# Arash-san/YinYang-Game-AlphaZero

Hardware: AMD Instinct MI355X
Metric: self-play positions/sec (+ MCTS node-expansions/sec) at 800 sims, 8x8 board (higher is better)
Workload: dtype f16x3; 1 GPU; 8x8 board, 800 sims/move, 4096 concurrent games per GPU, frozen random-init 128x10 net (seed 0), copied boards, reference_quirks=False, staggered start plies; tree_arithmetic=f32 PUCT + u64 bitboards, nn_dtype=f16x3, evaluation_reuse=False, parallelism=episode-sharded x1, lanes_per_gpu=2, hipgraph=True

## Files before the change

include/yy_engine.h:

```cpp
#ifndef YY_ENGINE_H
#define YY_ENGINE_H

#include <stdint.h>

#ifdef __cplusplus
extern "C" {
#endif

#define YY_OK 0
#define YY_E_INVALID (-1)
#define YY_E_UNSUPPORTED (-2)
#define YY_E_NOMEM (-3)
#define YY_E_HIP (-4)
#define YY_E_STATE (-5)
#define YY_E_ARENA (-6)

#define YY_FLAG_ROWCOL 1u
#define YY_FLAG_ALIASED 2u
#define YY_FLAG_REUSE_PASS_VALUE 4u

#define YY_FLAG_REUSE_TRANSPOSITIONS 8u
#define YY_FLAG_KEEP_EVALUATIONS 16u

typedef void *yy_stream_t;
// ... 59 lines not shown
int yy_mcts_root_counts(yy_mcts *ctx, int32_t *counts, float *child_w, float *child_p,
                        yy_stream_t stream);

int yy_mcts_root_policy(yy_mcts *ctx, int temperature_is_zero, double *pi, yy_stream_t stream);

int yy_mcts_root_stats(yy_mcts *ctx, int32_t *visits, double *value_sum, yy_stream_t stream);

int yy_mcts_get_boards(yy_mcts *ctx, int8_t *boards, yy_stream_t stream);

int yy_mcts_status(yy_mcts *ctx, int32_t *n_overflow, uint64_t *counters);
int yy_mcts_reset_counters(yy_mcts *ctx, yy_stream_t stream);
int yy_book_insert(const uint64_t *keys, int n, int R, int C, uint32_t *meta, uint64_t *table_keys, int64_t cap,
                   int32_t *slot_of, yy_stream_t stream);
int yy_mcts_set_book(yy_mcts *ctx, const uint32_t *meta, const uint64_t *keys, const float *value, const float *policy,
                     int64_t cap, int max_stones);
int yy_mcts_cache_clear(yy_mcts *ctx, yy_stream_t stream);

int yy_nn_bias_act_bf16(void *x, const float *bias, const void *residual, int64_t rows, int C,
                        int relu, yy_stream_t stream);

int yy_nn_tower_bf16(const float *planes, const void *weights, const float *bias, void *out, int G,
                     int R, int C, int channels, int n_layers, yy_stream_t stream);

int yy_nn_tower_heads_bf16(const float *planes, const void *weights, const float *bias,
                           void *out_heads, int G, int R, int C, int channels, int n_layers,
                           yy_stream_t stream);

int yy_nn_tower_f32(const float *planes, const void *weights, const float *bias, float *out, int G,
                    int R, int C, int channels, int n_layers, yy_stream_t stream);

int yy_nn_head_finish_bf16(const void *h, int G, int A, int H, const float *w2, const float *b2,
                           float *policy, float *value, yy_stream_t stream);

int yy_nn_tower_f16x3_regs(const float *planes, const void *weights, const void *head_w, const float *bias,
                           float *out, float *out_heads, const int32_t *rows, const int32_t *n_rows, int G,
                           int R, int C, int channels, int n_layers, int weight_exp, int head_exp,
                           int act_exp, yy_stream_t stream);

int yy_nn_tower_g(const float *planes, const void *weights, const void *head_w, const float *bias, const float *head_bias,
                  float *out, float *out_heads, const int32_t *rows, const int32_t *n_rows, int G, int R, int C,
                  int channels, int n_layers, int weight_exp, int head_exp, int act_exp, int nb, int boards, int gate_lo,
                  int gate_hi, int layout, yy_stream_t stream);
int yy_nn_tower_g_forms(int channels, int *nb_out);
int yy_nn_tower_g_relu_check(uint32_t start, uint32_t count, uint32_t *counts, yy_stream_t stream);

int yy_nn_fc_heads_f16x3(const float *feats, const void *wpk, const float *bias, const int32_t *jobs, int n_jobs,
                         float *logits, float *hidden, const int32_t *n_rows, int G, int K, int A, int H,
                         int weight_exp, int act_exp, yy_stream_t stream);

int yy_nn_head_finish_f32(const float *logits, const float *hidden, int G, int A, int H, const float *w2,
                          const float *b2, const int32_t *rows, const int32_t *n_rows, float *policy,
                          float *value, yy_stream_t stream);

int yy_compact_rows(const uint8_t *flags, int G, int32_t *rows, int32_t *n, yy_stream_t stream);

int yy_selfplay_root_noise(uint64_t seed, const int64_t *game_id, const int32_t *ply, const uint8_t *draw,
                           const uint8_t *mask, int G, int A, double alpha, double *noise, yy_stream_t stream);

int yy_selfplay_sample_actions(uint64_t seed, const int64_t *game_id, const int32_t *ply,
                               const uint8_t *searching, const double *pi, const uint8_t *mask, int G, int A,
                               int temperature_threshold, int32_t *action, yy_stream_t stream);

#ifdef __cplusplus
}
#endif
#endif
```

yinyang-game-alphazero_amd/_lib.py:

```python
import ctypes as C
import os
import subprocess

_HERE = os.path.dirname(os.path.abspath(__file__))
CSRC = os.path.join(_HERE, "csrc")
SO = os.path.join(CSRC, "libyy_hip.so")
HEADER = os.path.normpath(os.path.join(_HERE, "..", "include", "yy_engine.h"))

YY_OK = 0
YY_E_ARENA = -6
FLAG_ROWCOL = 1
FLAG_ALIASED = 2
FLAG_REUSE_PASS_VALUE = 4
FLAG_REUSE_TRANSPOSITIONS = 8
FLAG_KEEP_EVALUATIONS = 16

HIPCC_FLAGS = ["--offload-arch=gfx950", "-O3", "-std=c++17", "-fPIC", "-shared",
               "-ffp-contract=off", "-fno-fast-math", "-Wall", "-Wno-unused-function"]


class YYError(RuntimeError):
    def __init__(self, code, msg):
        super().__init__(f"libyy_hip: status {code}: {msg}")
        self.code = code
# ... 17 lines not shown
    if verbose:
        print(" ".join(cmd).replace(tmp, SO))
    try:
        subprocess.check_call(cmd)
        os.replace(tmp, SO)
    finally:
        if os.path.exists(tmp):
            os.remove(tmp)
    return SO


_LIB = None
_vp = C.c_void_p
_SIGS = {
    "yy_rules_valid_mask": [_vp, _vp, C.c_int, C.c_int, C.c_int, C.c_uint32, _vp, _vp],
    "yy_rules_step": [_vp, _vp, _vp, C.c_int, C.c_int, C.c_int, C.c_uint32, _vp, _vp],
    "yy_rules_game_ended": [_vp, _vp, C.c_int, C.c_int, C.c_int, C.c_uint32, _vp, _vp, _vp],
    "yy_encode_planes": [_vp, C.c_int, C.c_int, C.c_int, _vp, _vp],
    "yy_rules_mask_terminal_bb": [_vp, _vp, C.c_int, C.c_int, C.c_int, C.c_uint32, _vp, _vp, _vp, _vp],
    "yy_pack_boards": [_vp, C.c_int, C.c_int, C.c_int, _vp, _vp, _vp],
    "yy_unpack_boards": [_vp, _vp, C.c_int, C.c_int, C.c_int, _vp, _vp],
    "yy_mcts_create": [C.POINTER(MctsConfig), C.POINTER(_vp)],
    "yy_mcts_destroy": [_vp],
    "yy_mcts_memory_bytes": [_vp, C.POINTER(C.c_uint64)],
    "yy_mcts_set_num_sims": [_vp, C.c_int32],
    "yy_mcts_begin": [_vp, _vp, _vp, _vp, _vp, _vp],
    "yy_mcts_expand_root": [_vp, _vp, _vp, C.c_double, _vp],
    "yy_mcts_select": [_vp, _vp, _vp, _vp],
    "yy_mcts_expand_backup": [_vp, _vp, _vp, _vp],
    "yy_mcts_step": [_vp, _vp, _vp, _vp, _vp, _vp],
    "yy_mcts_root_counts": [_vp, _vp, _vp, _vp, _vp],
    "yy_mcts_root_policy": [_vp, C.c_int, _vp, _vp],
    "yy_mcts_root_stats": [_vp, _vp, _vp, _vp],
    "yy_mcts_get_boards": [_vp, _vp, _vp],
    "yy_mcts_status": [_vp, C.POINTER(C.c_int32), C.POINTER(C.c_uint64)],
    "yy_mcts_reset_counters": [_vp, _vp],
    "yy_mcts_cache_clear": [_vp, _vp],
    "yy_book_insert": [_vp, C.c_int, C.c_int, C.c_int, _vp, _vp, C.c_int64, _vp, _vp],
    "yy_mcts_set_book": [_vp, _vp, _vp, _vp, _vp, C.c_int64, C.c_int],
    "yy_nn_bias_act_bf16": [_vp, _vp, _vp, C.c_int64, C.c_int, C.c_int, _vp],
    "yy_nn_tower_bf16": [_vp, _vp, _vp, _vp, C.c_int, C.c_int, C.c_int, C.c_int, C.c_int, _vp],
    "yy_nn_tower_heads_bf16": [_vp, _vp, _vp, _vp, C.c_int, C.c_int, C.c_int, C.c_int, C.c_int, _vp],
    "yy_nn_head_finish_bf16": [_vp, C.c_int, C.c_int, C.c_int, _vp, _vp, _vp, _vp, _vp],
    "yy_nn_tower_f32": [_vp, _vp, _vp, _vp, C.c_int, C.c_int, C.c_int, C.c_int, C.c_int, _vp],
    "yy_nn_head_finish_f32": [_vp, _vp, C.c_int, C.c_int, C.c_int, _vp, _vp, _vp, _vp, _vp, _vp, _vp],
    "yy_compact_rows": [_vp, C.c_int, _vp, _vp, _vp],
    "yy_nn_tower_f16x3_regs": [_vp, _vp, _vp, _vp, _vp, _vp, _vp, _vp, C.c_int, C.c_int, C.c_int, C.c_int, C.c_int, C.c_int, C.c_int,
                               C.c_int, _vp],
    "yy_nn_tower_g_forms": [C.c_int, C.POINTER(C.c_int)],
    "yy_nn_tower_g_relu_check": [C.c_uint32, C.c_uint32, _vp, _vp],
    "yy_nn_tower_g": [_vp, _vp, _vp, _vp, _vp, _vp, _vp, _vp, _vp, C.c_int, C.c_int, C.c_int, C.c_int, C.c_int, C.c_int, C.c_int,
                      C.c_int, C.c_int, C.c_int, C.c_int, C.c_int, C.c_int, _vp],
    "yy_nn_fc_heads_f16x3": [_vp, _vp, _vp, _vp, C.c_int, _vp, _vp, _vp, C.c_int, C.c_int, C.c_int, C.c_int, C.c_int, C.c_int, _vp],
    "yy_selfplay_root_noise": [C.c_uint64, _vp, _vp, _vp, _vp, C.c_int, C.c_int, C.c_double, _vp, _vp],
    "yy_selfplay_sample_actions": [C.c_uint64, _vp, _vp, _vp, _vp, _vp, C.c_int, C.c_int, C.c_int, _vp, _vp],
    "yy_version": [],
}


def exported_symbols():
    return sorted(list(_SIGS) + ["yy_last_error"])


def lib():
    global _LIB
    if _LIB is None:
        if not os.path.exists(SO):
            raise YYError(-100, f"{SO} is missing: run __graft_entry__.build() (hipcc --offload-arch=gfx950); "
                                "there is no CPU fallback for the product path")
        L = C.CDLL(SO)
        for name, args in _SIGS.items():
            fn = getattr(L, name)
            fn.argtypes = args
            fn.restype = C.c_int
        L.yy_last_error.restype = C.c_char_p
        L.yy_last_error.argtypes = []
        _LIB = L
    return _LIB


def check(status):
    if status != YY_OK:
        raise YYError(status, lib().yy_last_error().decode())
    return status
```

yinyang-game-alphazero_amd/csrc/yy_common.h:

```cpp
#pragma once
#include <hip/hip_runtime.h>
#include <stdio.h>

#include "../../include/yy_engine.h"

extern "C" int yy_tower_set_err(int code, const char *msg);

static inline int yy_hip_fail(const char *what, hipError_t e) {
    char msg[512];
    snprintf(msg, sizeof msg, "%s: %s", what, hipGetErrorString(e));
    return yy_tower_set_err(YY_E_HIP, msg);
}
#define HIP_TRY(x)                                        \
    do {                                                  \
        hipError_t e_ = (x);                              \
        if (e_ != hipSuccess) return yy_hip_fail(#x, e_); \
    } while (0)

__device__ __forceinline__ float relu_keep_nan(float v) { return __builtin_isnan(v) ? v : fmaxf(v, 0.0f); }

template <int N> __device__ __forceinline__ void wait_vmcnt() { asm volatile("s_waitcnt vmcnt(%0)" ::"n"(N) : "memory"); }
```

yinyang-game-alphazero_amd/csrc/yy_fc_heads.hip:

```cpp
#include <hip/hip_runtime.h>
#include <math.h>
#include <stdint.h>

#include "../../include/yy_engine.h"

typedef __attribute__((ext_vector_type(8))) _Float16 f16x8;
typedef __attribute__((ext_vector_type(2))) _Float16 f16x2;
typedef __attribute__((ext_vector_type(4))) float f32x4;
typedef __attribute__((ext_vector_type(2))) float f32x2;
typedef __attribute__((ext_vector_type(4))) unsigned int u32x4;
typedef __attribute__((ext_vector_type(2))) unsigned int u32x2;

#include "yy_common.h"

namespace fch {

constexpr int KC = 128, RS = 288;

__device__ __forceinline__ void split_pair(const f32x2 a, uint32_t &hi, uint32_t &lo) {
    const f16x2 h = __builtin_convertvector(a, f16x2);
    const f32x2 r = a - __builtin_convertvector(h, f32x2);
    const f16x2 l = __builtin_convertvector(r, f16x2);
    hi = __builtin_bit_cast(uint32_t, h);
    lo = __builtin_bit_cast(uint32_t, l);
// ... 71 lines not shown
        __builtin_amdgcn_sched_group_barrier(0x100, 2 * P, 0);
#pragma unroll
        for (int g = 0; g < NG; g++) {
            const int ks = g / NBR, nb = g % NBR, slot = g % P;
            const f32x4 a = __builtin_amdgcn_mfma_f32_16x16x32_f16(w[ks][1], xh[slot], acc2[nb], 0, 0, 0);
            acc1[nb] = __builtin_amdgcn_mfma_f32_16x16x32_f16(w[ks][0], xh[slot], acc1[nb], 0, 0, 0);
            acc2[nb] = __builtin_amdgcn_mfma_f32_16x16x32_f16(w[ks][0], xl[slot], a, 0, 0, 0);
            if (g + P < NG) rd(g + P, slot);
            __builtin_amdgcn_sched_group_barrier(0x008, 3, 0);
            __builtin_amdgcn_sched_group_barrier(0x100, 2, 0);
        }
    };
    const int last = n_chunks - 1;
    f32x4 f0[NI], f1[NI];
    f16x8 w0[KC / 32][2], w1[KC / 32][2];
    stage_load(f1, 0);
    load_wc(w0, 0);
    stage_load(f0, min(1, last));
    load_wc(w1, min(1, last));
    stage_store(f1, 0);
    stage_load(f1, min(2, last));
    __syncthreads();
    for (int c = 0; c < n_chunks; c += 2) {
        compute(w0, 0);
        if (c + 1 < n_chunks) stage_store(f0, 1);
        stage_load(f0, min(c + 3, last));
        load_wc(w0, min(c + 2, last));
        __syncthreads();
        if (c + 1 >= n_chunks) break;
        compute(w1, 1);
        if (c + 2 < n_chunks) stage_store(f1, 0);
        stage_load(f1, min(c + 4, last));
        load_wc(w1, min(c + 3, last));
        __syncthreads();
    }
    if (!active) return;
    float *out = job.head == 0 ? logits : hidden;
    const int W = job.head == 0 ? A : H, boff = job.head == 0 ? 0 : A;
    const int o0 = job.out0 + wave * 16 + kg * 4;
    float b[4];
#pragma unroll
    for (int i = 0; i < 4; i++) b[i] = (o0 + i < job.out0 + job.nout) ? bias[boff + o0 + i] : 0.0f;
#pragma unroll
    for (int nb = 0; nb < NBR; nb++) {
        const int row = r0 + nb * 16 + n16;
        if (row < n_live) {
#pragma unroll
            for (int i = 0; i < 4; i++)
                if (o0 + i < job.out0 + job.nout) out[(size_t)row * W + o0 + i] = __builtin_fmaf(acc1[nb][i] + acc2[nb][i], out_scale, b[i]);
        }
    }
}

}

extern "C" int yy_nn_fc_heads_f16x3(const float *feats, const void *wpk, const float *bias, const int32_t *jobs, int n_jobs,
                                    float *logits, float *hidden, const int32_t *n_rows, int G, int K, int A, int H,
                                    int weight_exp, int act_exp, yy_stream_t s) {
    if (G == 0) return YY_OK;
    if (!feats || !wpk || !bias || !jobs || !logits || !hidden || G < 0 || n_jobs < 1 || K < 32 || (K & 31) || A < 1 || H < 1)
        return yy_tower_set_err(YY_E_INVALID, "yy_nn_fc_heads_f16x3: bad argument");
    const float in_scale = ldexpf(1.0f, act_exp), out_scale = ldexpf(1.0f, -(weight_exp + act_exp));
    if (G <= 2048)
        fch::k_fc_heads<32><<<dim3(((G + 31) / 32) * n_jobs), dim3(256), 0, (hipStream_t)s>>>(
            feats, (const unsigned char *)wpk, bias, (const fch::Job *)jobs, n_jobs, logits, hidden, n_rows, G, K, A, H, in_scale, out_scale);
    else
        fch::k_fc_heads<64><<<dim3(((G + 63) / 64) * n_jobs), dim3(256), 0, (hipStream_t)s>>>(
            feats, (const unsigned char *)wpk, bias, (const fch::Job *)jobs, n_jobs, logits, hidden, n_rows, G, K, A, H, in_scale, out_scale);
    if (hipGetLastError() != hipSuccess) return yy_tower_set_err(YY_E_HIP, "yy_nn_fc_heads_f16x3: launch failed");
    return YY_OK;
}
```

yinyang-game-alphazero_amd/csrc/yy_nn_epilogue.hip:

```cpp
#include <hip/hip_runtime.h>
#include <math.h>
#include <stdint.h>

#include "../../include/yy_engine.h"
#include "yy_common.h"

typedef __attribute__((ext_vector_type(8))) unsigned short us8;

__device__ __forceinline__ float bf2f(unsigned short h) { return __uint_as_float(((uint32_t)h) << 16); }
__device__ __forceinline__ unsigned short f2bf(float f) {
    uint32_t u = __float_as_uint(f);
    if ((u & 0x7FFFFFFFu) > 0x7F800000u) return (unsigned short)((u >> 16) | 0x40u);
    return (unsigned short)((u + 0x7FFFu + ((u >> 16) & 1u)) >> 16);
}

template <bool HAS_RES, bool RELU, bool FIXED>
__global__ void __launch_bounds__(256) k_bias_act(us8 *x, const float *bias, const us8 *res, size_t n_vec, int cvec) {
    const size_t tid = (size_t)blockIdx.x * blockDim.x + threadIdx.x;
    const size_t stride = (size_t)gridDim.x * blockDim.x;
    float b[8];
    if (FIXED) {
        const float4 *bp = reinterpret_cast<const float4 *>(bias + (tid % (size_t)cvec) * 8);
        const float4 b0 = bp[0], b1 = bp[1];
        b[0] = b0.x; b[1] = b0.y; b[2] = b0.z; b[3] = b0.w;
// ... 27 lines not shown
        if (relu) k_bias_act<true, true, FIXED><<<dim3(blocks), dim3(256), 0, st>>>(xv, bias, rv, n_vec, cvec);
        else k_bias_act<true, false, FIXED><<<dim3(blocks), dim3(256), 0, st>>>(xv, bias, rv, n_vec, cvec);
    } else {
        if (relu) k_bias_act<false, true, FIXED><<<dim3(blocks), dim3(256), 0, st>>>(xv, bias, rv, n_vec, cvec);
        else k_bias_act<false, false, FIXED><<<dim3(blocks), dim3(256), 0, st>>>(xv, bias, rv, n_vec, cvec);
    }
}

extern "C" int yy_nn_bias_act_bf16(void *x, const float *bias, const void *residual, int64_t rows, int C, int relu,
                                   yy_stream_t s) {
    if (rows == 0) return YY_OK;
    if (!x || !bias || rows < 0 || C <= 0) return yy_tower_set_err(YY_E_INVALID, "bad argument");
    if (C % 8) return yy_tower_set_err(YY_E_UNSUPPORTED, "channels must be a multiple of 8");
    const int cvec = C / 8;
    const size_t n_vec = (size_t)rows * (size_t)cvec;
    size_t blocks = (n_vec + 255) / 256;
    if (blocks > 256 * 8) blocks = 256 * 8;
    const bool fixed = (256 % cvec) == 0;
    if (fixed) launch_bias_act<true>((us8 *)x, bias, (const us8 *)residual, n_vec, cvec, relu, (unsigned)blocks, (hipStream_t)s);
    else launch_bias_act<false>((us8 *)x, bias, (const us8 *)residual, n_vec, cvec, relu, (unsigned)blocks, (hipStream_t)s);
    HIP_TRY(hipGetLastError());
    return YY_OK;
}

__global__ void __launch_bounds__(64) k_head_finish(const unsigned short *__restrict__ h, int A, int H,
                                                    const float *__restrict__ w2, const float *__restrict__ b2,
                                                    float *__restrict__ policy, float *__restrict__ value) {
    const int g = blockIdx.x, lane = threadIdx.x;
    const unsigned short *row = h + (size_t)g * (A + H);
    float mx = -INFINITY;
    for (int a = lane; a < A; a += 64) mx = fmaxf(mx, bf2f(row[a]));
#pragma unroll
    for (int o = 32; o > 0; o >>= 1) mx = fmaxf(mx, __shfl_xor(mx, o, 64));
    float sum = 0.0f;
    for (int a = lane; a < A; a += 64) sum += expf(bf2f(row[a]) - mx);
#pragma unroll
    for (int o = 32; o > 0; o >>= 1) sum += __shfl_xor(sum, o, 64);
    for (int a = lane; a < A; a += 64) policy[(size_t)g * A + a] = expf(bf2f(row[a]) - mx) / sum;
    float acc = 0.0f;
    for (int j = lane; j < H; j += 64) acc += fmaxf(bf2f(row[A + j]), 0.0f) * w2[j];
#pragma unroll
    for (int o = 32; o > 0; o >>= 1) acc += __shfl_xor(acc, o, 64);
    if (lane == 0) value[g] = tanhf(acc + b2[0]);
}

__global__ void __launch_bounds__(64) k_head_finish_f32(const float *__restrict__ logits, const float *__restrict__ hidden,
                                                        int A, int H, const float *__restrict__ w2,
                                                        const float *__restrict__ b2, const int32_t *__restrict__ rows,
                                                        const int32_t *__restrict__ n_rows, float *__restrict__ policy,
                                                        float *__restrict__ value) {
    const int i = blockIdx.x, lane = threadIdx.x;
    if (n_rows && i >= *n_rows) return;
    const int g = rows ? rows[i] : i;
    const float *row = logits + (size_t)i * A;
    float mx = -INFINITY;
    for (int a = lane; a < A; a += 64) mx = fmaxf(mx, row[a]);
#pragma unroll
    for (int o = 32; o > 0; o >>= 1) mx = fmaxf(mx, __shfl_xor(mx, o, 64));
    float sum = 0.0f;
    for (int a = lane; a < A; a += 64) sum += expf(row[a] - mx);
#pragma unroll
    for (int o = 32; o > 0; o >>= 1) sum += __shfl_xor(sum, o, 64);
    for (int a = lane; a < A; a += 64) policy[(size_t)g * A + a] = expf(row[a] - mx) / sum;
    const float *hr = hidden + (size_t)i * H;
    float acc = 0.0f;
    for (int j = lane; j < H; j += 64) acc += relu_keep_nan(hr[j]) * w2[j];
#pragma unroll
    for (int o = 32; o > 0; o >>= 1) acc += __shfl_xor(acc, o, 64);
    if (lane == 0) value[g] = tanhf(acc + b2[0]);
}

extern "C" int yy_nn_head_finish_f32(const float *logits, const float *hidden, int G, int A, int H, const float *w2,
                                     const float *b2, const int32_t *rows, const int32_t *n_rows, float *policy, float *value,
                                     yy_stream_t s) {
    if (G == 0) return YY_OK;
    if (!logits || !hidden || !w2 || !b2 || !policy || !value || G < 0 || A <= 0 || H <= 0 || (rows && !n_rows))
        return yy_tower_set_err(YY_E_INVALID, "bad argument");
    k_head_finish_f32<<<dim3(G), dim3(64), 0, (hipStream_t)s>>>(logits, hidden, A, H, w2, b2, rows, n_rows, policy, value);
    HIP_TRY(hipGetLastError());
    return YY_OK;
}

__global__ void __launch_bounds__(1024) k_compact_rows(const uint8_t *__restrict__ flags, int G, int32_t *__restrict__ rows,
                                                       int32_t *__restrict__ n) {
    __shared__ int wsum[16];
    const int t = threadIdx.x, lane = t & 63, wave = t >> 6;
    const int per = (G + 1023) / 1024, lo = min(t * per, G), hi = min(lo + per, G);
    int cnt = 0;
    for (int g = lo; g < hi; g++) cnt += flags[g] != 0;
    int incl = cnt;
#pragma unroll
    for (int o = 1; o < 64; o <<= 1) {
        const int v = __shfl_up(incl, o, 64);
        if (lane >= o) incl += v;
    }
    if (lane == 63) wsum[wave] = incl;
    __syncthreads();
    int base = 0;
    for (int w = 0; w < wave; w++) base += wsum[w];
    int pos = base + incl - cnt;
    for (int g = lo; g < hi; g++)
        if (flags[g] != 0) rows[pos++] = g;
    if (t == 1023) *n = base + incl;
}

extern "C" int yy_compact_rows(const uint8_t *flags, int G, int32_t *rows, int32_t *n, yy_stream_t s) {
    if (!flags || !rows || !n || G < 0) return yy_tower_set_err(YY_E_INVALID, "bad argument");
    k_compact_rows<<<dim3(1), dim3(1024), 0, (hipStream_t)s>>>(flags, G, rows, n);
    HIP_TRY(hipGetLastError());
    return YY_OK;
}

extern "C" int yy_nn_head_finish_bf16(const void *h, int G, int A, int H, const float *w2, const float *b2, float *policy,
                                      float *value, yy_stream_t s) {
    if (G == 0) return YY_OK;
    if (!h || !w2 || !b2 || !policy || !value || G < 0 || A <= 0 || H <= 0) return yy_tower_set_err(YY_E_INVALID, "bad argument");
    k_head_finish<<<dim3(G), dim3(64), 0, (hipStream_t)s>>>((const unsigned short *)h, A, H, w2, b2, policy, value);
    HIP_TRY(hipGetLastError());
    return YY_OK;
}
```

yinyang-game-alphazero_amd/engine.py:

```python
import ctypes as ct

import torch

from . import _lib
from ._lib import FLAG_ALIASED, FLAG_REUSE_PASS_VALUE, FLAG_KEEP_EVALUATIONS, FLAG_REUSE_TRANSPOSITIONS, FLAG_ROWCOL, MctsConfig, check, lib


def _stream():
    return ct.c_void_p(torch.cuda.current_stream().cuda_stream)


def _p(t):
    return None if t is None else ct.c_void_p(t.data_ptr())


def _need(t, dtype, shape=None, name="tensor"):
    if not isinstance(t, torch.Tensor) or not t.is_cuda:
        raise _lib.YYError(-1, f"{name}: expected a ROCm device tensor (the hot path has no CPU fallback)")
    if t.dtype != dtype or not t.is_contiguous():
        raise _lib.YYError(-1, f"{name}: expected contiguous {dtype}, got {t.dtype} contiguous={t.is_contiguous()}")
    if shape is not None and tuple(t.shape) != tuple(shape):
        raise _lib.YYError(-1, f"{name}: expected shape {tuple(shape)}, got {tuple(t.shape)}")
    return t

# ... 175 lines not shown
    with torch.cuda.device(planes.device):
        check(lib().yy_nn_tower_g(_p(planes), _p(weights), _p(head_w), _p(bias), _p(head_bias), None if heads else _p(out),
                                  _p(out) if heads else None, _p(rows), _p(n_rows), G, R, Cc, ch, n_layers, int(exps[0]), int(exps[1]),
                                  int(exps[2]), int(nb), int(boards), int(gate[0]), int(gate[1]),
                                  1 if column_layout else 0 if wave_grid else 2,
                                  _stream()))
    return out if heads else out.permute(0, 3, 1, 2)


def tower_g_relu_check(start, count, counts):
    _need(counts, torch.int32, (2,), "counts")
    with torch.cuda.device(counts.device):
        check(lib().yy_nn_tower_g_relu_check(int(start) & 0xFFFFFFFF, int(count), _p(counts), _stream()))
    return counts


def fc_heads(feats, wpk, bias, jobs, A, H, exps, n_rows=None, logits=None, hidden=None):
    G, two, K = feats.shape
    _need(feats, torch.float32, (G, 2, K), "feats")
    _need(jobs, torch.int32, (jobs.shape[0], 4), "jobs")
    ksteps = ((K + 127) // 128) * 4
    _need(wpk, torch.int16, (jobs.shape[0] * ksteps * 4096,), "fc head weights (pack_fc_heads)")
    _need(bias, torch.float32, (A + H,), "fc head bias")
    if n_rows is not None:
        _need(n_rows, torch.int32, (1,), "n_rows")
    if logits is None:
        logits = torch.empty((G, A), dtype=torch.float32, device=feats.device)
        hidden = torch.empty((G, H), dtype=torch.float32, device=feats.device)
    _need(logits, torch.float32, (G, A), "logits")
    _need(hidden, torch.float32, (G, H), "hidden")
    with torch.cuda.device(feats.device):
        check(lib().yy_nn_fc_heads_f16x3(_p(feats), _p(wpk), _p(bias), _p(jobs), jobs.shape[0], _p(logits), _p(hidden), _p(n_rows), G, K,
                                         A, H, int(exps[0]), int(exps[1]), _stream()))
    return logits, hidden


def head_finish_f32(logits, hidden, w2, b2, rows=None, n_rows=None, policy=None, value=None):
    G, A = logits.shape
    _need(logits, torch.float32, name="logits")
    _need(hidden, torch.float32, (G, hidden.shape[1]), "hidden")
    _need(w2, torch.float32, (hidden.shape[1],), "w2")
    _need(b2, torch.float32, (1,), "b2")
    if rows is not None:
        _need(rows, torch.int32, (G,), "rows")
        _need(n_rows, torch.int32, (1,), "n_rows")
    if policy is None:
        policy = torch.zeros((G, A), dtype=torch.float32, device=logits.device)
        value = torch.zeros(G, dtype=torch.float32, device=logits.device)
    _need(policy, torch.float32, (G, A), "policy")
    _need(value, torch.float32, (G,), "value")
    with torch.cuda.device(logits.device):
        check(lib().yy_nn_head_finish_f32(_p(logits), _p(hidden), G, A, hidden.shape[1], _p(w2), _p(b2), _p(rows), _p(n_rows),
                                          _p(policy), _p(value), _stream()))
    return policy, value


def compact_rows(flags, rows=None, n=None):
    G = flags.shape[0]
    _need(flags, torch.uint8, (G,), "flags")
    if rows is None:
        rows = torch.zeros(G, dtype=torch.int32, device=flags.device)
        n = torch.zeros(1, dtype=torch.int32, device=flags.device)
    _need(rows, torch.int32, (G,), "rows")
    _need(n, torch.int32, (1,), "n")
    with torch.cuda.device(flags.device):
        check(lib().yy_compact_rows(_p(flags), G, _p(rows), _p(n), _stream()))
    return rows, n


def tower_heads_forward(planes, weights, bias, n_layers):
    G, _, R, Cc = planes.shape
    _need(planes, torch.float32, (G, 5, R, Cc), "planes")
    n_chunks = 9 + 18 * (n_layers - 1) + 1
    _need(weights, torch.int16, (n_chunks, 8192), "tower+heads weights")
    _need(bias, torch.float32, (n_layers + 1, 128), "tower+heads bias")
    out = torch.empty((G, 2, 32 * R * Cc), dtype=torch.bfloat16, device=planes.device)
    with torch.cuda.device(planes.device):
        check(lib().yy_nn_tower_heads_bf16(_p(planes), _p(weights), _p(bias), _p(out), G, R, Cc, 128, n_layers, _stream()))
    return out


def head_finish(h, A, w2, b2):
    G, W = h.shape
    _need(h, torch.bfloat16, name="h")
    _need(w2, torch.float32, (W - A,), "w2")
    _need(b2, torch.float32, (1,), "b2")
    policy = torch.empty((G, A), dtype=torch.float32, device=h.device)
    value = torch.empty(G, dtype=torch.float32, device=h.device)
    with torch.cuda.device(h.device):
        check(lib().yy_nn_head_finish_bf16(_p(h), G, A, W - A, _p(w2), _p(b2), _p(policy), _p(value), _stream()))
    return policy, value


def root_noise(seed, game_id, ply, draw, mask, alpha):
    G, A = mask.shape
    _need(game_id, torch.int64, (G,), "game_id")
    _need(ply, torch.int32, (G,), "ply")
    _need(draw, torch.uint8, (G,), "draw")
    _need(mask, torch.uint8, (G, A), "mask")
    out = torch.empty((G, A), dtype=torch.float64, device=mask.device)
    with torch.cuda.device(mask.device):
        check(lib().yy_selfplay_root_noise(ct.c_uint64(int(seed) & (2 ** 64 - 1)), _p(game_id), _p(ply), _p(draw), _p(mask), G, A,
                                           float(alpha), _p(out), _stream()))
    return out


# ... 252 lines not shown
```

yinyang-game-alphazero_amd/network.py:

```python
import os

import numpy as np
import torch
import torch.nn as nn
import torch.nn.functional as F

from . import engine

H3_BOARDS = ((6, 6), (8, 8), (12, 12))
G_MAX_CELLS = 144
G_CHANNELS = (32, 64, 96, 128)
G_SPLIT_WG = 256
G_HINT_BIG_ONLY = 4
G_AUTO_MAX_WG = 2048
HEAD_CHANNELS = 32
VALUE_HIDDEN = 256
INPUT_PLANES = 5


class ResidualBlock(nn.Module):

    def __init__(self, channels):
        super().__init__()
        for i in (1, 2):
            setattr(self, f"conv{i}", nn.Conv2d(channels, channels, 3, padding=1))
            setattr(self, f"bn{i}", nn.BatchNorm2d(channels))

    def forward(self, x):
        y = F.relu(self.bn1(self.conv1(x)))
        y = self.bn2(self.conv2(y))
        return F.relu(y + x)


class YinYangNeuralNetwork(nn.Module):
    def __init__(self, game, num_channels=128, num_res_blocks=10):
        super().__init__()
        self.game = game
        self.board_size = tuple(game.getBoardSize())
        self.action_size = game.getActionSize()
        self.input_channels = INPUT_PLANES
        cells = self.board_size[0] * self.board_size[1]
        self.conv1 = nn.Conv2d(INPUT_PLANES, num_channels, 3, padding=1)
        self.bn1 = nn.BatchNorm2d(num_channels)
        self.res_blocks = nn.ModuleList(ResidualBlock(num_channels) for _ in range(num_res_blocks))
        self.policy_conv = nn.Conv2d(num_channels, HEAD_CHANNELS, 1)
        self.policy_bn = nn.BatchNorm2d(HEAD_CHANNELS)
        self.policy_fc = nn.Linear(HEAD_CHANNELS * cells, self.action_size)
        self.value_conv = nn.Conv2d(num_channels, HEAD_CHANNELS, 1)
        self.value_bn = nn.BatchNorm2d(HEAD_CHANNELS)
        self.value_fc1 = nn.Linear(HEAD_CHANNELS * cells, VALUE_HIDDEN)
        self.value_fc2 = nn.Linear(VALUE_HIDDEN, 1)
        for mod in self.modules():
            if isinstance(mod, (nn.Conv2d, nn.Linear)):
                nn.init.xavier_normal_(mod.weight)
                if mod.bias is not None:
                    nn.init.zeros_(mod.bias)

    def forward(self, x):
        x = F.relu(self.bn1(self.conv1(x)))
        for blk in self.res_blocks:
            x = blk(x)
        p = F.relu(self.policy_bn(self.policy_conv(x))).flatten(1)
        v = F.relu(self.value_bn(self.value_conv(x))).flatten(1)
        return self.policy_fc(p), torch.tanh(self.value_fc2(F.relu(self.value_fc1(v))))

    @torch.no_grad()
    def predict_batch(self, planes):
# ... 247 lines not shown
            mode = reference_precision_mode(net)
        self.mode = mode
        self.device = next(net.parameters()).device
        self.supports_compaction = False
        self.supports_static = False
        self.row_independent = False
        self.fused = self.tower = self.fused_heads = self.use_h3r = False
        self.g_split = None
        self._hint = {}
        self._static = {}
        if mode in ("f16x3", "f16x3r"):
            self._init_split_f16(net, mode == "f16x3r")
            self._forward = BatchedEvaluator._forward_split_f16
        elif mode == "fp32t":
            self._init_fp32t(net)
            self._forward = BatchedEvaluator._forward_fp32t
        elif mode == "fp32":
            self._forward = BatchedEvaluator._forward_fp32
        else:
            self._init_reduced(net, {"bf16": torch.bfloat16, "fp16": torch.float16}[mode], fused_epilogue, tower, fused_heads)
            self._forward = BatchedEvaluator._forward_reduced

    @torch.no_grad()
    def __call__(self, planes, needs_eval=None, static=False):
        if needs_eval is not None and not self.supports_compaction:
            raise ValueError(f"evaluator mode {self.mode} does not take needs_eval")
        return self._forward(self, planes, needs_eval, static)

    def form_key(self, owner):
        hint = self._hint.get(owner)
        if hint is None or self.g_split is None:
            return 0
        return 1 if hint >= 2 * self.g_split else 0

    def rows_hint(self, owner, mean_rows):
        self._hint[owner] = float(mean_rows)

    def _init_split_f16(self, net, h3r):
        if not f16x3_covers(net):
            raise ValueError("f16x3 needs a board of at most 144 cells, 32/64/96/128 channels, at most 10 residual blocks, 32-channel heads")
        dev = self.device
        R, C = net.board_size
        self.h3_layers = 1 + 2 * len(net.res_blocks)
        wq, bq, kw = pack_tower_g(net)
        hw, hb, kh = pack_heads_g(net)
        self.g_w, self.g_b, self.g_hw, self.g_hb = wq.to(dev), bq.to(dev), hw.to(dev), hb.to(dev)
        self.g_exps = (kw, kh, ACT_EXP)
        self.g_big, self.g_small = tower_g_forms(R * C, net.conv1.out_channels)
        self.g_split = G_SPLIT_WG * self.g_small[1]
        fw, fb, jobs, kf = pack_fc_heads(net)
        self.fc_w, self.fc_b, self.fc_jobs, self.fc_exps = fw.to(dev), fb.to(dev), jobs.to(dev), (kf, ACT_EXP)
        self.n_actions, self.n_hidden = net.policy_fc.out_features, net.value_fc1.out_features
        self.fc2_w, self.fc2_b = fc2_vector(net)
        if h3r:
            if tuple(net.board_size) not in H3_BOARDS or net.conv1.out_channels != 128:
                raise ValueError("f16x3r needs 6x6, 8x8 or 12x12 boards and 128 channels")
            wr, br, kw_r = pack_tower_h3r(net)
            hr, hbr, kh_r = pack_heads_h3r(net)
            self.h3r_w, self.h3r_hw = wr.to(dev), hr.to(dev)
            self.h3_b = torch.cat([br, hbr]).contiguous().to(dev)
            self.h3_exps = (kw_r, kh_r, ACT_EXP)
            self.use_h3r = True
            self.mode = "f16x3"
        self.supports_compaction = self.supports_static = True
        self.row_independent = True

    def _form_plan(self, G, compacted, owner):
        big, small, split, ungated = self.g_big, self.g_small, self.g_split, (-1, 0x7FFFFFFF)
        if small == big or G > G_AUTO_MAX_WG * small[1]:
            return [(big, ungated)]
        if G <= split:
            return [(small, ungated)]
        if not compacted:
            return [(big, ungated)]
        hint = self._hint.get(owner) if owner is not True and owner is not False else None
        if hint is not None and hint >= G_HINT_BIG_ONLY * split:
            return [(big, ungated)]
        return [(small, (-1, split)), (big, (split, 0x7FFFFFFF))]

    def _forward_split_f16(self, planes, needs_eval, static):
        G = planes.shape[0]
        K = 32 * planes.shape[2] * planes.shape[3]
        rows = n = pol = val = feats = logits = hidden = None
        if static:
            key = (G, 0 if static is True else static)
            buf = self._static.get(key)
            if buf is None:
                dev = planes.device
                z = lambda shape, dt=torch.float32: torch.zeros(shape, dtype=dt, device=dev)
                buf = self._static[key] = (z(G, torch.int32), z(1, torch.int32), z((G, self.n_actions)), z(G), z((G, 2, K)),
                                         z((G, self.n_actions)), z((G, self.n_hidden)))
            rows, n, pol, val, feats, logits, hidden = buf
        if needs_eval is not None:
            rows, n = engine.compact_rows(needs_eval, rows, n)
        else:
            rows = n = None
        if self.use_h3r:
            feats = engine.tower_heads_forward_h3r(planes, self.h3r_w, self.h3r_hw, self.h3_b, self.h3_layers, self.h3_exps, rows, n, feats)
        else:
            for form, gate in self._form_plan(G, rows is not None, static):
                feats = engine.tower_g(planes, self.g_w, self.g_b, self.h3_layers, self.g_exps, form[0], form[1],
                                       self.g_hw, self.g_hb, rows, n, feats, gate)
        logits, hidden = engine.fc_heads(feats, self.fc_w, self.fc_b, self.fc_jobs, self.n_actions, self.n_hidden, self.fc_exps, n,
                                         logits, hidden)
        return engine.head_finish_f32(logits, hidden, self.fc2_w, self.fc2_b, rows, n, pol, val)

    def _forward_fp32(self, planes, needs_eval, static):
        return self.net.predict_batch(planes)

    def _init_fp32t(self, net):
        if tuple(net.board_size) != (8, 8) or net.conv1.out_channels != 128 or len(net.res_blocks) > 11:
            raise ValueError(self.mode + " needs 8x8 boards, 128 channels, at most 11 residual blocks")
        wq, bq = pack_tower_f32(net)
        self.f32_w, self.f32_b = wq.to(self.device), bq.to(self.device)
        self.f32_layers = 1 + 2 * len(net.res_blocks)
        hw, hb = folded_head_convs(net)
        self.hconv_w, self.hconv_b = hw.t().contiguous().to(self.device), hb.to(self.device)
        wc, bc = fc_block(net)
        self.fc_cat_w, self.fc_cat_b = wc.contiguous(), bc.contiguous()
        w2, self.fc2_b = fc2_vector(net)
        self.fc2_w = w2.reshape(-1, 1)
        self.n_actions = net.policy_fc.out_features

    def _forward_fp32t(self, planes, needs_eval, static):
        x = engine.tower_forward_f32(planes, self.f32_w, self.f32_b, self.f32_layers)
        G = x.shape[0]
        cells = x.shape[2] * x.shape[3]
        hc = torch.addmm(self.hconv_b, x.permute(0, 2, 3, 1).reshape(G * cells, -1), self.hconv_w)
        feats = torch.relu_(hc).view(G, cells, -1).transpose(1, 2).reshape(G, -1)
        h = torch.addmm(self.fc_cat_b, feats, self.fc_cat_w.t())
        A = self.n_actions
        value = torch.tanh(torch.addmm(self.fc2_b, torch.relu(h[:, A:]), self.fc2_w)).reshape(-1)
        return F.softmax(h[:, :A], dim=1), value

    def _init_reduced(self, net, dtype, fused_epilogue, tower, fused_heads):
        self.dtype = dtype
        self.fused = bool(fused_epilogue) and self.mode == "bf16"
        self._fold()
        self.tower = (bool(tower) and self.mode == "bf16" and tuple(net.board_size) in ((6, 6), (8, 8), (12, 12))
                      and net.conv1.out_channels == 128 and len(net.res_blocks) <= 10)
        if not self.tower:
            return
        wq, bq = pack_tower(net)
        self.tower_w, self.tower_b = wq.to(self.device), bq.to(self.device)
        self.tower_layers = 1 + 2 * len(net.res_blocks)
        self.fused_heads = bool(fused_heads) and net.policy_conv.out_channels == 32
        if self.fused_heads:
            hw, hb = pack_heads(net)
            self.towerh_w = torch.cat([wq, hw]).contiguous().to(self.device)
            self.towerh_b = torch.cat([bq, hb]).contiguous().to(self.device)
            wc, bc = fc_block(net)
            self.fc_cat_w, self.fc_cat_b = wc.to(dtype).contiguous(), bc.to(dtype).contiguous()
            self.fc2_w, self.fc2_b = fc2_vector(net)
            self.n_actions = net.policy_fc.out_features

# ... 44 lines not shown
```

Before: 1826 positions/s.

## Fuse FC heads GEMM with softmax/value finish in one kernel

Adds a kernel that runs the policy/value FC-head MFMA GEMM over row tiles and then, without leaving the block, does the softmax and value tanh from LDS. It writes policy and value directly. This removes one kernel launch and the global-memory round trip for the logits and hidden buffers. In exchange, each block handles a whole row tile across all output columns with launch_bounds(256,1), which may lower parallelism compared with the separate FC kernel.

```diff
diff --git a/include/yy_engine.h b/include/yy_engine.h
--- a/include/yy_engine.h
+++ b/include/yy_engine.h
@@ -135,6 +135,13 @@
                           const float *b2, const int32_t *rows, const int32_t *n_rows, float *policy,
                           float *value, yy_stream_t stream);
 
+int yy_nn_fc_heads_finish_f16x3(const float *feats, const void *wpk, const float *bias, const int32_t *jobs, int n_jobs,
+                                const float *w2, const float *b2, const int32_t *rows, const int32_t *n_rows,
+                                float *policy, float *value, int G, int K, int A, int H, int weight_exp, int act_exp,
+                                int tile, yy_stream_t stream);
+
+int yy_nn_fc_heads_finish_tiles(int A, int H, int *tiles);
+
 int yy_compact_rows(const uint8_t *flags, int G, int32_t *rows, int32_t *n, yy_stream_t stream);
 
 int yy_selfplay_root_noise(uint64_t seed, const int64_t *game_id, const int32_t *ply, const uint8_t *draw,
diff --git a/yinyang-game-alphazero_amd/_lib.py b/yinyang-game-alphazero_amd/_lib.py
--- a/yinyang-game-alphazero_amd/_lib.py
+++ b/yinyang-game-alphazero_amd/_lib.py
@@ -93,6 +93,9 @@
     "yy_nn_tower_g": [_vp, _vp, _vp, _vp, _vp, _vp, _vp, _vp, _vp, C.c_int, C.c_int, C.c_int, C.c_int, C.c_int, C.c_int, C.c_int,
                       C.c_int, C.c_int, C.c_int, C.c_int, C.c_int, C.c_int, _vp],
     "yy_nn_fc_heads_f16x3": [_vp, _vp, _vp, _vp, C.c_int, _vp, _vp, _vp, C.c_int, C.c_int, C.c_int, C.c_int, C.c_int, C.c_int, _vp],
+    "yy_nn_fc_heads_finish_f16x3": [_vp, _vp, _vp, _vp, C.c_int, _vp, _vp, _vp, _vp, _vp, _vp, C.c_int, C.c_int, C.c_int, C.c_int, C.c_int,
+                                    C.c_int, C.c_int, _vp],
+    "yy_nn_fc_heads_finish_tiles": [C.c_int, C.c_int, C.POINTER(C.c_int)],
     "yy_selfplay_root_noise": [C.c_uint64, _vp, _vp, _vp, _vp, C.c_int, C.c_int, C.c_double, _vp, _vp],
     "yy_selfplay_sample_actions": [C.c_uint64, _vp, _vp, _vp, _vp, _vp, C.c_int, C.c_int, C.c_int, _vp, _vp],
     "yy_version": [],
diff --git a/yinyang-game-alphazero_amd/csrc/yy_common.h b/yinyang-game-alphazero_amd/csrc/yy_common.h
--- a/yinyang-game-alphazero_amd/csrc/yy_common.h
+++ b/yinyang-game-alphazero_amd/csrc/yy_common.h
@@ -1,5 +1,6 @@
 #pragma once
 #include <hip/hip_runtime.h>
+#include <math.h>
 #include <stdio.h>
 
 #include "../../include/yy_engine.h"
@@ -19,4 +20,23 @@
 
 __device__ __forceinline__ float relu_keep_nan(float v) { return __builtin_isnan(v) ? v : fmaxf(v, 0.0f); }
 
+__device__ __forceinline__ void head_finish_row(const float *row, const float *hr, int A, int H, const float *__restrict__ w2,
+                                                const float *__restrict__ b2, float *__restrict__ policy_row,
+                                                float *__restrict__ value, int lane) {
+    float mx = -INFINITY;
+    for (int a = lane; a < A; a += 64) mx = fmaxf(mx, row[a]);
+#pragma unroll
+    for (int o = 32; o > 0; o >>= 1) mx = fmaxf(mx, __shfl_xor(mx, o, 64));
+    float sum = 0.0f;
+    for (int a = lane; a < A; a += 64) sum += expf(row[a] - mx);
+#pragma unroll
+    for (int o = 32; o > 0; o >>= 1) sum += __shfl_xor(sum, o, 64);
+    for (int a = lane; a < A; a += 64) policy_row[a] = expf(row[a] - mx) / sum;
+    float acc = 0.0f;
+    for (int j = lane; j < H; j += 64) acc += relu_keep_nan(hr[j]) * w2[j];
+#pragma unroll
+    for (int o = 32; o > 0; o >>= 1) acc += __shfl_xor(acc, o, 64);
+    if (lane == 0) *value = tanhf(acc + b2[0]);
+}
+
 template <int N> __device__ __forceinline__ void wait_vmcnt() { asm volatile("s_waitcnt vmcnt(%0)" ::"n"(N) : "memory"); }
diff --git a/yinyang-game-alphazero_amd/csrc/yy_fc_heads.hip b/yinyang-game-alphazero_amd/csrc/yy_fc_heads.hip
--- a/yinyang-game-alphazero_amd/csrc/yy_fc_heads.hip
+++ b/yinyang-game-alphazero_amd/csrc/yy_fc_heads.hip
@@ -147,6 +147,132 @@
     }
 }
 
+template <int ROWS, int NP, int RING>
+__global__ void __launch_bounds__(256, 1)
+k_fc_heads_finish(const float *__restrict__ feats, const unsigned char *__restrict__ wpk, const float *__restrict__ bias,
+                  const Job *__restrict__ jobs, const float *__restrict__ w2, const float *__restrict__ b2,
+                  const int32_t *__restrict__ rows, const int *__restrict__ n_rows, float *__restrict__ policy,
+                  float *__restrict__ value, int G, int K, int A, float in_scale, float out_scale) {
+    constexpr int NV = 4, NM = NP + NV, H = 64 * NV, NBR = ROWS / 16, NI = ROWS / 8;
+    constexpr int PART_BYTES = ROWS * RS, HEAD_BYTES = 2 * PART_BYTES, STAGE_BYTES = 2 * HEAD_BYTES;
+    constexpr int FW = H + 64 * NP + 4;
+    static_assert(4 % RING == 0 && ROWS * FW * 4 <= 2 * STAGE_BYTES, "ring / finish tile");
+    __shared__ __attribute__((aligned(256))) unsigned char lds[2 * STAGE_BYTES];
+    const int n_live = n_rows ? min(*n_rows, G) : G;
+    const int r0 = blockIdx.x * ROWS;
+    if (r0 >= n_live) return;
+    const int lane = threadIdx.x & 63, wave = __builtin_amdgcn_readfirstlane(threadIdx.x >> 6);
+    const int n16 = lane & 15, kg = lane >> 4;
+    const int n_chunks = (K + KC - 1) / KC, last = n_chunks - 1, last_ks = 4 * n_chunks - 1;
+
+    const int sq = threadIdx.x & 31, sr = threadIdx.x >> 5;
+    auto stage_load = [&](f32x4 (&fr)[2][NI], float &km, int c) {
+        const int k = c * KC + sq * 4;
+        const int kc = k < K ? k : 0;
+        km = k < K ? 1.0f : 0.0f;
+#pragma unroll
+        for (int i = 0; i < NI; i++) {
+            const int row = min(r0 + sr + 8 * i, n_live - 1);
+            const float *p = feats + (size_t)row * 2 * K + kc;
+            fr[0][i] = *(const f32x4 *)p;
+            fr[1][i] = *(const f32x4 *)(p + K);
+        }
+    };
+    auto stage_store = [&](const f32x4 (&fr)[2][NI], float km, int s) {
+        unsigned char *base = lds + s * STAGE_BYTES + sq * 8;
+#pragma unroll
+        for (int hd = 0; hd < 2; hd++)
+#pragma unroll
+            for (int i = 0; i < NI; i++) {
+                const f32x4 v = fr[hd][i] * km * in_scale;
+                uint32_t h01, l01, h23, l23;
+                split_pair((f32x2){v[0], v[1]}, h01, l01);
+                split_pair((f32x2){v[2], v[3]}, h23, l23);
+                *(u32x2 *)(base + hd * HEAD_BYTES + (sr + 8 * i) * RS) = (u32x2){h01, h23};
+                *(u32x2 *)(base + hd * HEAD_BYTES + PART_BYTES + (sr + 8 * i) * RS) = (u32x2){l01, l23};
+            }
+    };
+    int wch[NM];
+#pragma unroll
+    for (int mb = 0; mb < NM; mb++) wch[mb] = __builtin_amdgcn_readfirstlane(jobs[mb].wchunk);
+    const unsigned char *wlane = wpk + wave * 2048 + lane * 16;
+    auto load_w = [&](f16x8 (&w)[NM][2], int ks) {
+#pragma unroll
+        for (int mb = 0; mb < NM; mb++) {
+            const unsigned char *p = wlane + (size_t)(wch[mb] + ks) * 8192;
+            w[mb][0] = __builtin_bit_cast(f16x8, *(const u32x4 *)p);
+            w[mb][1] = __builtin_bit_cast(f16x8, *(const u32x4 *)(p + 1024));
+        }
+    };
+    f32x4 acc1[NM][NBR], acc2[NM][NBR];
+#pragma unroll
+    for (int mb = 0; mb < NM; mb++)
+#pragma unroll
+        for (int nb = 0; nb < NBR; nb++) acc1[mb][nb] = acc2[mb][nb] = (f32x4){0.f, 0.f, 0.f, 0.f};
+    auto compute = [&](const f16x8 (&w)[NM][2], int stage, int ks) {
+        const unsigned char *xs = lds + stage * STAGE_BYTES + n16 * RS + kg * 16 + ks * 64;
+#pragma unroll
+        for (int hd = 0; hd < 2; hd++) {
+            f16x8 xh[NBR], xl[NBR];
+#pragma unroll
+            for (int nb = 0; nb < NBR; nb++) {
+                xh[nb] = __builtin_bit_cast(f16x8, *(const u32x4 *)(xs + hd * HEAD_BYTES + nb * 16 * RS));
+                xl[nb] = __builtin_bit_cast(f16x8, *(const u32x4 *)(xs + hd * HEAD_BYTES + PART_BYTES + nb * 16 * RS));
+            }
+#pragma unroll
+            for (int mb = (hd == 0 ? 0 : NP); mb < (hd == 0 ? NP : NM); mb++)
+#pragma unroll
+                for (int nb = 0; nb < NBR; nb++) {
+                    const f32x4 a = __builtin_amdgcn_mfma_f32_16x16x32_f16(w[mb][1], xh[nb], acc2[mb][nb], 0, 0, 0);
+                    acc1[mb][nb] = __builtin_amdgcn_mfma_f32_16x16x32_f16(w[mb][0], xh[nb], acc1[mb][nb], 0, 0, 0);
+                    acc2[mb][nb] = __builtin_amdgcn_mfma_f32_16x16x32_f16(w[mb][0], xl[nb], a, 0, 0, 0);
+                }
+        }
+    };
+    f16x8 wr[RING][NM][2];
+    f32x4 fr[2][NI];
+    float km;
+#pragma unroll
+    for (int r = 0; r < RING; r++) load_w(wr[r], min(r, last_ks));
+    stage_load(fr, km, 0);
+    stage_store(fr, km, 0);
+    stage_load(fr, km, min(1, last));
+    __syncthreads();
+    for (int c = 0; c < n_chunks; c++) {
+        const int st = c & 1;
+#pragma unroll
+        for (int ks = 0; ks < KC / 32; ks++) {
+            compute(wr[ks % RING], st, ks);
+            load_w(wr[ks % RING], min(c * (KC / 32) + ks + RING, last_ks));
+        }
+        if (c + 1 < n_chunks) stage_store(fr, km, st ^ 1);
+        stage_load(fr, km, min(c + 2, last));
+        __syncthreads();
+    }
+    float *fin = (float *)lds;
+#pragma unroll
+    for (int mb = 0; mb < NM; mb++) {
+        const int o0 = (mb < NP ? mb : mb - NP) * 64 + wave * 16 + kg * 4;
+        const int W = mb < NP ? A : H, boff = mb < NP ? 0 : A, col = mb < NP ? H + o0 : o0;
+        float b[4];
+#pragma unroll
+        for (int i = 0; i < 4; i++) b[i] = (o0 + i < W) ? bias[boff + o0 + i] : 0.0f;
+#pragma unroll
+        for (int nb = 0; nb < NBR; nb++) {
+            f32x4 v;
+#pragma unroll
+            for (int i = 0; i < 4; i++) v[i] = __builtin_fmaf(acc1[mb][nb][i] + acc2[mb][nb][i], out_scale, b[i]);
+            *(f32x4 *)(fin + (nb * 16 + n16) * FW + col) = v;
+        }
+    }
+    __syncthreads();
+    const int n_tile = min(ROWS, n_live - r0);
+    for (int r = wave; r < n_tile; r += 4) {
+        const int i = r0 + r, g = rows ? rows[i] : i;
+        head_finish_row(fin + r * FW + H, fin + r * FW, A, H, w2, b2, policy + (size_t)g * A, value + g, lane);
+    }
+}
+
 }
 
 extern "C" int yy_nn_fc_heads_f16x3(const float *feats, const void *wpk, const float *bias, const int32_t *jobs, int n_jobs,
@@ -165,3 +291,53 @@
     if (hipGetLastError() != hipSuccess) return yy_tower_set_err(YY_E_HIP, "yy_nn_fc_heads_f16x3: launch failed");
     return YY_OK;
 }
+
+extern "C" int yy_nn_fc_heads_finish_tiles(int A, int H, int *tiles) {
+    if (H != 256 || A < 1 || A > 192) return 0;
+    const int n = A <= 128 ? 2 : 1;
+    if (tiles) {
+        tiles[0] = 32;
+        if (n > 1) tiles[1] = 64;
+    }
+    return n;
+}
+
+template <int ROWS, int RING>
+static void launch_fc_heads_finish(int np, int G, hipStream_t st, const float *feats, const unsigned char *wpk, const float *bias,
+                                   const fch::Job *jobs, const float *w2, const float *b2, const int32_t *rows, const int32_t *n_rows,
+                                   float *policy, float *value, int K, int A, float in_scale, float out_scale) {
+    const dim3 grid((G + ROWS - 1) / ROWS), block(256);
+    if (np == 1)
+        fch::k_fc_heads_finish<ROWS, 1, RING><<<grid, block, 0, st>>>(feats, wpk, bias, jobs, w2, b2, rows, n_rows, policy, value, G, K, A, in_scale, out_scale);
+    else if (np == 2)
+        fch::k_fc_heads_finish<ROWS, 2, RING><<<grid, block, 0, st>>>(feats, wpk, bias, jobs, w2, b2, rows, n_rows, policy, value, G, K, A, in_scale, out_scale);
+    else if constexpr (ROWS == 32)
+        fch::k_fc_heads_finish<ROWS, 3, RING><<<grid, block, 0, st>>>(feats, wpk, bias, jobs, w2, b2, rows, n_rows, policy, value, G, K, A, in_scale, out_scale);
+}
+
+extern "C" int yy_nn_fc_heads_finish_f16x3(const float *feats, const void *wpk, const float *bias, const int32_t *jobs, int n_jobs,
+                                           const float *w2, const float *b2, const int32_t *rows, const int32_t *n_rows,
+                                           float *policy, float *value, int G, int K, int A, int H, int weight_exp, int act_exp,
+                                           int tile, yy_stream_t s) {
+    if (G == 0) return YY_OK;
+    if (!feats || !wpk || !bias || !jobs || !w2 || !b2 || !policy || !value || G < 0 || K < 32 || (K & 31) || A < 1 || H < 1 ||
+        (rows && !n_rows))
+        return yy_tower_set_err(YY_E_INVALID, "yy_nn_fc_heads_finish_f16x3: bad argument");
+    int tiles[4];
+    const int n_tiles = yy_nn_fc_heads_finish_tiles(A, H, tiles);
+    if (!n_tiles) return yy_tower_set_err(YY_E_UNSUPPORTED, "yy_nn_fc_heads_finish_f16x3: needs H = 256 and A <= 192");
+    if (tile != 0 && tile != tiles[0] && !(n_tiles > 1 && tile == tiles[1]))
+        return yy_tower_set_err(YY_E_INVALID, "yy_nn_fc_heads_finish_f16x3: tile is not one of yy_nn_fc_heads_finish_tiles");
+    const int np = (A + 63) / 64;
+    if (n_jobs != np + 4) return yy_tower_set_err(YY_E_INVALID, "yy_nn_fc_heads_finish_f16x3: jobs are not pack_fc_heads's for (A, H)");
+    const float in_scale = ldexpf(1.0f, act_exp), out_scale = ldexpf(1.0f, -(weight_exp + act_exp));
+    if (tile == 0) tile = 32;
+    if (tile == 32)
+        launch_fc_heads_finish<32, 4>(np, G, (hipStream_t)s, feats, (const unsigned char *)wpk, bias, (const fch::Job *)jobs, w2, b2, rows,
+                                      n_rows, policy, value, K, A, in_scale, out_scale);
+    else
+        launch_fc_heads_finish<64, 2>(np, G, (hipStream_t)s, feats, (const unsigned char *)wpk, bias, (const fch::Job *)jobs, w2, b2, rows,
+                                      n_rows, policy, value, K, A, in_scale, out_scale);
+    if (hipGetLastError() != hipSuccess) return yy_tower_set_err(YY_E_HIP, "yy_nn_fc_heads_finish_f16x3: launch failed");
+    return YY_OK;
+}
diff --git a/yinyang-game-alphazero_amd/csrc/yy_nn_epilogue.hip b/yinyang-game-alphazero_amd/csrc/yy_nn_epilogue.hip
--- a/yinyang-game-alphazero_amd/csrc/yy_nn_epilogue.hip
+++ b/yinyang-game-alphazero_amd/csrc/yy_nn_epilogue.hip
@@ -103,22 +103,7 @@
     const int i = blockIdx.x, lane = threadIdx.x;
     if (n_rows && i >= *n_rows) return;
     const int g = rows ? rows[i] : i;
-    const float *row = logits + (size_t)i * A;
-    float mx = -INFINITY;
-    for (int a = lane; a < A; a += 64) mx = fmaxf(mx, row[a]);
-#pragma unroll
-    for (int o = 32; o > 0; o >>= 1) mx = fmaxf(mx, __shfl_xor(mx, o, 64));
-    float sum = 0.0f;
-    for (int a = lane; a < A; a += 64) sum += expf(row[a] - mx);
-#pragma unroll
-    for (int o = 32; o > 0; o >>= 1) sum += __shfl_xor(sum, o, 64);
-    for (int a = lane; a < A; a += 64) policy[(size_t)g * A + a] = expf(row[a] - mx) / sum;
-    const float *hr = hidden + (size_t)i * H;
-    float acc = 0.0f;
-    for (int j = lane; j < H; j += 64) acc += relu_keep_nan(hr[j]) * w2[j];
-#pragma unroll
-    for (int o = 32; o > 0; o >>= 1) acc += __shfl_xor(acc, o, 64);
-    if (lane == 0) value[g] = tanhf(acc + b2[0]);
+    head_finish_row(logits + (size_t)i * A, hidden + (size_t)i * H, A, H, w2, b2, policy + (size_t)g * A, value + g, lane);
 }
 
 extern "C" int yy_nn_head_finish_f32(const float *logits, const float *hidden, int G, int A, int H, const float *w2,
diff --git a/yinyang-game-alphazero_amd/engine.py b/yinyang-game-alphazero_amd/engine.py
--- a/yinyang-game-alphazero_amd/engine.py
+++ b/yinyang-game-alphazero_amd/engine.py
@@ -251,6 +251,37 @@
     with torch.cuda.device(logits.device):
         check(lib().yy_nn_head_finish_f32(_p(logits), _p(hidden), G, A, hidden.shape[1], _p(w2), _p(b2), _p(rows), _p(n_rows),
                                           _p(policy), _p(value), _stream()))
+    return policy, value
+
+
+def fc_heads_finish_tiles(A, H):
+    buf = (ct.c_int * 4)()
+    n = lib().yy_nn_fc_heads_finish_tiles(int(A), int(H), buf)
+    return [int(buf[i]) for i in range(n)]
+
+
+def fc_heads_finish(feats, wpk, bias, jobs, A, H, exps, w2, b2, rows=None, n_rows=None, policy=None, value=None, tile=0):
+    G, two, K = feats.shape
+    _need(feats, torch.float32, (G, 2, K), "feats")
+    _need(jobs, torch.int32, (jobs.shape[0], 4), "jobs")
+    ksteps = ((K + 127) // 128) * 4
+    _need(wpk, torch.int16, (jobs.shape[0] * ksteps * 4096,), "fc head weights (pack_fc_heads)")
+    _need(bias, torch.float32, (A + H,), "fc head bias")
+    _need(w2, torch.float32, (H,), "w2")
+    _need(b2, torch.float32, (1,), "b2")
+    if n_rows is not None:
+        _need(n_rows, torch.int32, (1,), "n_rows")
+    if rows is not None:
+        _need(rows, torch.int32, (G,), "rows")
+    if policy is None:
+        policy = torch.zeros((G, A), dtype=torch.float32, device=feats.device)
+        value = torch.zeros(G, dtype=torch.float32, device=feats.device)
+    _need(policy, torch.float32, (G, A), "policy")
+    _need(value, torch.float32, (G,), "value")
+    with torch.cuda.device(feats.device):
+        check(lib().yy_nn_fc_heads_finish_f16x3(_p(feats), _p(wpk), _p(bias), _p(jobs), jobs.shape[0], _p(w2), _p(b2), _p(rows),
+                                                _p(n_rows), _p(policy), _p(value), G, K, A, H, int(exps[0]), int(exps[1]), int(tile),
+                                                _stream()))
     return policy, value
 
 
diff --git a/yinyang-game-alphazero_amd/network.py b/yinyang-game-alphazero_amd/network.py
--- a/yinyang-game-alphazero_amd/network.py
+++ b/yinyang-game-alphazero_amd/network.py
@@ -13,6 +13,7 @@
 G_SPLIT_WG = 256
 G_HINT_BIG_ONLY = 4
 G_AUTO_MAX_WG = 2048
+FC_FINISH_FUSED = True
 HEAD_CHANNELS = 32
 VALUE_HIDDEN = 256
 INPUT_PLANES = 5
@@ -366,6 +367,7 @@
         self.fc_w, self.fc_b, self.fc_jobs, self.fc_exps = fw.to(dev), fb.to(dev), jobs.to(dev), (kf, ACT_EXP)
         self.n_actions, self.n_hidden = net.policy_fc.out_features, net.value_fc1.out_features
         self.fc2_w, self.fc2_b = fc2_vector(net)
+        self.fc_finish = bool(FC_FINISH_FUSED and dev.type == "cuda" and engine.fc_heads_finish_tiles(self.n_actions, self.n_hidden))
         if h3r:
             if tuple(net.board_size) not in H3_BOARDS or net.conv1.out_channels != 128:
                 raise ValueError("f16x3r needs 6x6, 8x8 or 12x12 boards and 128 channels")
@@ -402,8 +404,8 @@
             if buf is None:
                 dev = planes.device
                 z = lambda shape, dt=torch.float32: torch.zeros(shape, dtype=dt, device=dev)
-                buf = self._static[key] = (z(G, torch.int32), z(1, torch.int32), z((G, self.n_actions)), z(G), z((G, 2, K)),
-                                         z((G, self.n_actions)), z((G, self.n_hidden)))
+                two = (None, None) if self.fc_finish else (z((G, self.n_actions)), z((G, self.n_hidden)))
+                buf = self._static[key] = (z(G, torch.int32), z(1, torch.int32), z((G, self.n_actions)), z(G), z((G, 2, K))) + two
             rows, n, pol, val, feats, logits, hidden = buf
         if needs_eval is not None:
             rows, n = engine.compact_rows(needs_eval, rows, n)
@@ -415,6 +417,9 @@
             for form, gate in self._form_plan(G, rows is not None, static):
                 feats = engine.tower_g(planes, self.g_w, self.g_b, self.h3_layers, self.g_exps, form[0], form[1],
                                        self.g_hw, self.g_hb, rows, n, feats, gate)
+        if self.fc_finish:
+            return engine.fc_heads_finish(feats, self.fc_w, self.fc_b, self.fc_jobs, self.n_actions, self.n_hidden, self.fc_exps,
+                                          self.fc2_w, self.fc2_b, rows, n, pol, val)
         logits, hidden = engine.fc_heads(feats, self.fc_w, self.fc_b, self.fc_jobs, self.n_actions, self.n_hidden, self.fc_exps, n,
                                          logits, hidden)
         return engine.head_finish_f32(logits, hidden, self.fc2_w, self.fc2_b, rows, n, pol, val)
```

Result: no change. 1825 positions/s (-0.1%).
